# nelpy/ghost

Measured on AMD Instinct MI355X. Metric: Msamples/s CWT (128ch x 1e6 samp x 100 scales); % HBM roofline; 1/2/4/8 GPU, higher is better.
Workload: dtype f32

## Files before the change

ghost_amd/csrc/api.cpp:

```cpp
#include <hip/hip_runtime.h>

#include <algorithm>
#include <cmath>
#include <cstdio>
#include <cstdlib>
#include <cstring>
#include <exception>
#include <map>
#include <new>
#include <string>
#include <vector>

#include "../../include/ghostcwt.h"
#include "../../include/ghostcwt_debug.h"
#include <memory>

#include "errors.h"
#include "host_out.h"
#include "interp.h"
#include "kernels.h"
#include "morse_exact.h"
#include "morlet_exact.h"
#include "options.h"
#include "planner.h"
// ... 12 lines not shown

int hip_err(hipError_t e, const char* what) {
  g_err = std::string(what) + ": " + hipGetErrorString(e);
  return e == hipErrorOutOfMemory ? GCWT_ERR_NOMEM : GCWT_ERR_HIP;
}

#define HIP_TRY(call)                                  \
  do {                                                 \
    hipError_t e_ = (call);                            \
    if (e_ != hipSuccess) return hip_err(e_, #call);   \
  } while (0)

struct EpochDev {
  SynthItemDev* items = nullptr;
  int n_items = 0;
  SynthLevelDev* levels = nullptr;
  Synth7Item* items7 = nullptr;
  Synth7Level* levels7 = nullptr;
  int n_items7 = 0;
  Synth7Item* items7w = nullptr;
  int n_items7w = 0;
  Synth7Item* items7n = nullptr;
  int n_items7n = 0;
  SynthiItem* items_i = nullptr;
  SynthiLevel* levels_i = nullptr;
  int n_items_i = 0;
  SynthpItem* items_p[2] = {nullptr, nullptr};
  SynthpLevel* levels_p = nullptr;
  int n_items_p[2] = {0, 0};
  PredLevel* pred_levels = nullptr;
};

constexpr int64_t kFullbandCacheBytes = (int64_t)16 << 30;

enum Stage { ST_MEAN = 0, ST_FWD, ST_DECIM, ST_BLOCK, ST_SYNTH, ST_DIRECT, ST_FULLBAND, ST_INTERP, ST_BLOCKCONV, ST_COUNT };

}

struct gcwt_plan {
  HostPlan hp;
  bool uploaded = false;
  int profiling = 0;
  int synth_cols = 32;
  int synth7_narrow_r = 2;
  bool fuse_blocks = true;
  int synth_kernel = 7;
  bool prune_inputs = true;
  bool fast_fft = true;
  int drop_stores = 0;
  bool clock_probe = false;
  bool use_synth16 = false;
  int device = -1;
  hipStream_t stream = nullptr;
  hipStream_t aux[2] = {nullptr, nullptr};
  bool level_streams = true;
  bool use_synthp = false;
  bool use_graphs = true;
  bool fullband4 = true;
  int fullband_group = 0;
  int64_t fullband_cache_cap = 0;
  bool hfull_cache_full = false;
  int synth7_order = 0;
  int synthp_help = -1;
  int synthp_lgnb = -1;
  int interp_lgnb = -1;
  int interp_grid = -1;
  bool last_fold = false;
// ... 102 lines not shown

template <typename T>
int upload_vec(T** p, const std::vector<T>& v, hipStream_t st) {
  int rc = dev_alloc(p, v.size());
  if (rc) return rc;
  if (!v.empty()) HIP_TRY(hipMemcpyAsync(*p, v.data(), v.size() * sizeof(T), hipMemcpyHostToDevice, st));
  return GCWT_OK;
}

void free_dev(gcwt_plan* p) {
  auto fr = [](auto*& q) { if (q) { (void)hipFree((void*)q); q = nullptr; } };
  fr(p->d_y); fr(p->d_tw64); fr(p->d_x); fr(p->d_xr); fr(p->d_xb); fr(p->d_xs); fr(p->d_probe); fr(p->d_amps); fr(p->d_z); fr(p->d_hfull); fr(p->d_bank); fr(p->d_gain); fr(p->d_gain_lv); fr(p->d_half_tw); fr(p->d_psi); fr(p->d_psi_tail); fr(p->d_psi_lit); fr(p->d_tw4096);
  fr(p->d_tw256); fr(p->d_level_tw); fr(p->d_sums); fr(p->d_scale_list); fr(p->d_scale_aux); fr(p->d_interp_coef); fr(p->d_bank_sc); fr(p->d_direct_sc); fr(p->d_bc_h); fr(p->d_bc_rows); fr(p->d_bc_x); fr(p->d_bc_tw);
  fr(p->d_in);
  if (p->d_out) { (void)hipFree(p->d_out); p->d_out = nullptr; }
  if (p->h_pred) { (void)hipHostFree(p->h_pred); p->h_pred = nullptr; }
  fr(p->d_hist); fr(p->d_bands); fr(p->d_pred); fr(p->d_scale_level); fr(p->d_scale_length); fr(p->d_run_mask);
  for (gcwt_plan*& sub : p->sub_plan)
    if (sub) { gcwt_plan_destroy(sub); sub = nullptr; }
  for (auto& kv : p->hfull_cache) (void)hipFree(kv.second);
  p->hfull_cache.clear();
  p->hfull_cache_bytes = 0;
  p->host_out.release();
  for (auto& e : p->ep_dev) { fr(e.items); fr(e.levels); fr(e.items7); fr(e.items7w); fr(e.items7n); fr(e.levels7); fr(e.items_i); fr(e.levels_i); fr(e.items_p[0]); fr(e.items_p[1]); fr(e.levels_p); fr(e.pred_levels); }
  p->ep_dev.clear();
  if (p->graph_exec) { (void)hipGraphExecDestroy(p->graph_exec); p->graph_exec = nullptr; }
  for (auto e : p->ev_pool) (void)hipEventDestroy(e);
  p->ev_pool.clear();
  if (p->stream) { (void)hipStreamDestroy(p->stream); p->stream = nullptr; }
  for (auto& q : p->aux) if (q) { (void)hipStreamDestroy(q); q = nullptr; }
  if (p->det_stream) { (void)hipStreamDestroy(p->det_stream); p->det_stream = nullptr; }
  p->uploaded = false;
}

int get_event(gcwt_plan* p, hipEvent_t* e) {
  if (p->ev_used == p->ev_pool.size()) {
    hipEvent_t n;
    HIP_TRY(hipEventCreate(&n));
    p->ev_pool.push_back(n);
  }
  *e = p->ev_pool[p->ev_used++];
  return GCWT_OK;
}

enum LevelKernel { LK_SYNTH16 = 0, LK_SYNTH7 = 7, LK_INTERP = 9 };
inline bool level_pipelined(const gcwt_plan* p, const LevelPlan& lp) {
  return p->use_synthp && lp.interp_q == 2 && lp.interp_factor >= 4 && lp.interp_factor <= kSynthpMaxFactor &&
// ... 110 lines not shown
      return set_err(GCWT_ERR_INVALID, "a destination that is not page-locked takes dense rows (dst_pitch = row_elems)");
    HIP_TRY(rows_to_host(d_src, src_pitch, n_rows, row_elems, dst, dst_pitch, (flags & GCWT_OUT_F64) != 0,
                         (flags & GCWT_HOST_PINNED) != 0));
    return (int)GCWT_OK;
  });
}

static int gcwt_plan_create_impl(gcwt_plan** out, const gcwt_params* params) {
  if (!out || !params) return set_err(GCWT_ERR_INVALID, "NULL argument");
  *out = nullptr;
  std::unique_ptr<gcwt_plan> owner(new (std::nothrow) gcwt_plan());
  gcwt_plan* p = owner.get();
  if (!p) return set_err(GCWT_ERR_NOMEM, "out of host memory");
  std::string err;
  int rc = build_host_plan(*params, &p->hp, &err);
  if (rc != GCWT_OK) return set_err(rc, err);
  p->hp.prm.freqs_hz = p->hp.freqs.data();
  p->hp.prm.epoch_bounds = p->hp.bounds.data();
  p->hp.prm.n_epochs = (int32_t)(p->hp.bounds.size() / 2);
  p->device = params->device;
  p->high_precision = p->hp.high_precision;
  p->use_synth16 = option_or("synth16", 0) == 1;
  p->synth_cols = option_or("synth_cols", 32) == 16 ? 16 : 32;
  p->synth7_narrow_r = (int)option_or("synth7_narrow_r", 2);
  p->fuse_blocks = option_or("fuse_blocks", 1) != 0;
  p->prune_inputs = option_or("prune_inputs", 1) != 0;
  p->fast_fft = option_or("slow_fft", 0) == 0;
  p->level_streams = option_or("level_streams", 1) != 0;
  if (option_is_set("interp_grid")) p->interp_grid = option_or("interp_grid", 0) != 0;
  p->synth_streams = option_or("synth_streams", 0) != 0;
  p->fold_mean = option_or("fold_mean", 1) != 0;
  p->interp_lgnb = (int)option_or("interp_lgnb", -1);
  p->use_synthp = kMeasureBuild && option_or("synthp", 0) != 0;
  p->synthp_lgnb = (int)option_or("synthp_lgnb", -1);
  p->synthp_help = (int)option_or("synthp_help", -1);
  p->use_graphs = option_or("graphs", 1) != 0;
  p->synth7_order = (int)option_or("synth7_order", 0);
  p->auto_threshold = 1e-9f * (float)option_or("auto_threshold_ppb", 1500);
  p->kappa_eps = 1e-9f * (float)option_or("auto_kappa_ppb", 160);
  p->oob_tol = 1e-12f * (float)option_or("auto_oob_ppt", 25000);
  p->fullband_group = (int)option_or("fullband_group", 0);
  p->fullband4 = option_or("fullband4", 1) != 0;
  p->synth_kernel = kMeasureBuild && option_or("synth_kernel", 7) == 8 ? 8 : 7;
  p->drop_stores = kMeasureBuild && option_is_set("synth_drop_stores") ? (int)std::max<long long>(1, option_or("synth_drop_stores", 1)) : 0;
  p->clock_probe = kMeasureBuild && option_is_set("clock_probe");
  for (const auto& s : p->hp.scales)
    if (s.method == GCWT_SCALE_DIRECT) p->max_direct_len = std::max(p->max_direct_len, s.length);
// ... 273 lines not shown
  if ((rc = upload_vec(&p->d_interp_coef, hp.interp_coef, p->stream))) return bail(rc);
  p->n_listed = (int)scale_list.size();
  {
    const size_t n = ((size_t)p->n_listed + 8) * 256 * (hp.morlet ? 2 : 1);
    if ((rc = dev_alloc(&p->d_gain_lv, n))) return bail(rc);
    hipError_t hz = hipMemsetAsync(p->d_gain_lv, 0, sizeof(float) * n, p->stream);
    if (hz != hipSuccess) return bail(hip_err(hz, "gain rows reset"));
  }
  p->ep_dev.resize(hp.epochs.size());
  for (size_t e = 0; e < hp.epochs.size(); ++e) {
    const EpochPlan& ep = hp.epochs[e];
    if (ep.batch_count == 0) continue;
    std::vector<SynthItemDev> items;
    for (size_t i = 0; i < ep.items.size(); ++i)
      if (level_kernel(p, hp.levels[ep.items[i].level]) == LK_SYNTH16)
        items.push_back({ep.items[i].level, ep.items[i].scale, ep.items[i].blk0, ep.items[i].nblk});
    p->ep_dev[e].n_items = (int)items.size();
    std::vector<SynthLevelDev> lv(hp.levels.size());
    for (size_t l = 0; l < lv.size(); ++l)
      lv[l] = {hp.levels[l].decimation, hp.levels[l].hop, hp.levels[l].halo, ep.lv[l].blk_lo,
               ep.lv[l].xb_offset, hp.levels[l].twiddle_offset};
    if ((rc = upload_vec(&p->ep_dev[e].items, items, p->stream))) return bail(rc);
    if ((rc = upload_vec(&p->ep_dev[e].levels, lv, p->stream))) return bail(rc);
    std::vector<Synth7Item> items7, items7w, items7n;
    std::vector<Synth7Level> lv7(hp.levels.size());
    for (size_t l = 0; l < lv7.size(); ++l) {
      const LevelPlan& lp = hp.levels[l];
      int lg = 0;
      while ((1 << lg) < lp.decimation) ++lg;
      lv7[l] = {lp.decimation, lg, lp.hop, lp.halo, ep.lv[l].nblk, (int32_t)lp.scales.size(),
                scale_off[l], ep.lv[l].blk_lo, n_plain[l], (int32_t)(l * 256), lp.band_shift, 0, ep.lv[l].xb_offset,
                lp.twiddle_offset, ep.lv[l].xr_offset, ep.lv[l].m - 1};
      const bool narrow = lp.halo <= 48 && lp.decimation <= p->synth7_narrow_r && p->synth_cols == 32;
      const int cols = narrow ? 16 : p->synth_cols;
      const int bpb = std::max(1, cols / lp.decimation);
      const int n_rtiles = std::max(1, lp.decimation / cols);
      if (level_kernel(p, lp) != LK_SYNTH7) continue;
      for (int b0 = 0; b0 < ep.lv[l].nblk; b0 += bpb)
        for (int rt = 0; rt < n_rtiles; ++rt) (lp.halo > 48 ? items7w : narrow ? items7n : items7).push_back({(int32_t)l, b0, rt, 0});
    }
    if (p->synth7_order == 1) std::reverse(items7.begin(), items7.end());
    else if (p->synth7_order == 2) {
      std::vector<std::vector<Synth7Item>> by(hp.levels.size());
      for (const auto& it : items7) by[(size_t)it.level].push_back(it);
      std::vector<Synth7Item> mixed;
      std::vector<double> pos(by.size(), 0.0);
      size_t left = items7.size();
      while (left) {
        size_t best = by.size(); double frac = 2.0;
        for (size_t l = 0; l < by.size(); ++l)
          if (pos[l] < (double)by[l].size() && pos[l] / (double)by[l].size() < frac) { frac = pos[l] / (double)by[l].size(); best = l; }
        mixed.push_back(by[best][(size_t)pos[best]]);
        pos[best] += 1.0; --left;
      }
      items7.swap(mixed);
    }
    p->ep_dev[e].n_items7 = (int)items7.size();
    p->ep_dev[e].n_items7w = (int)items7w.size();
    p->ep_dev[e].n_items7n = (int)items7n.size();
    if ((rc = upload_vec(&p->ep_dev[e].items7n, items7n, p->stream))) return bail(rc);
    if ((rc = upload_vec(&p->ep_dev[e].items7, items7, p->stream))) return bail(rc);
    if ((rc = upload_vec(&p->ep_dev[e].items7w, items7w, p->stream))) return bail(rc);
    if ((rc = upload_vec(&p->ep_dev[e].levels7, lv7, p->stream))) return bail(rc);
    std::vector<SynthiItem> items_i;
    std::vector<std::pair<int, int>> pending;
    std::vector<SynthiLevel> lvi(hp.levels.size());
    std::vector<int> order;
    std::vector<int> order_p;
    for (size_t l = 0; l < hp.levels.size(); ++l)
      if (level_kernel(p, hp.levels[l]) == LK_INTERP)
        (level_pipelined(p, hp.levels[l]) ? order_p : order).push_back((int)l);
    std::sort(order.begin(), order.end(),
              [&](int x, int y) { return hp.levels[x].decimation > hp.levels[y].decimation; });
    std::sort(order_p.begin(), order_p.end(),
              [&](int x, int y) { return hp.levels[x].decimation > hp.levels[y].decimation; });
    for (int l : order) {
      const LevelPlan& lp = hp.levels[l];
      int lgq = 0;
      while ((1 << lgq) < lp.interp_q) ++lgq;
      int lgnb = lp.decimation <= 32 && lp.interp_q <= 2 ? 1 : 0;
      if (p->interp_lgnb >= 0) lgnb = std::min(p->interp_lgnb, 2);
      while (lgnb > 0 && (lp.interp_q << lgnb) > kInterpMaxPhases) --lgnb;
// ... 369 lines not shown
        RUN(ST_DECIM, launch_level_small(p->d_x, xr, n1, q, kRowLen, P, hp.max_xr, p->d_tw4096, slots, ls, taper));
      }
      const float scale = (float)(1.0 / ((double)hp.block * (double)Pt));
      const LevelKernel lk = level_kernel(p, lp);
      if (lk == LK_SYNTH16 || (lk == LK_SYNTH7 && !fused_blocks))
        RUN(ST_BLOCK, launch_block_fft(xr, p->d_xb + el.xb_offset, el.m, lp.hop, lp.halo, el.blk_lo,
                                       el.nblk, hp.max_xr, hp.max_xb, p->d_tw256, scale, slots, ls));
    }
    if (side) {
      p->cur = nullptr;
      for (int k = 0; k < 2; ++k) {
        if (!forked[k]) continue;
        hipEvent_t done;
        int rc_ = get_event(p, &done);
        if (rc_) return rc_;
        he = hipEventRecord(done, p->aux[k]);
        if (he == hipSuccess) he = hipStreamWaitEvent(st, done, 0);
        if (he != hipSuccess) return hip_err(he, "level streams join");
      }
    }
    const EpochDev& dev = p->ep_dev[ep.batch_first];
    hipStream_t si = st;
    if (dev.n_items_i > 0) {
      const bool beside = p->synth_streams && (dev.n_items7 > 0 || dev.n_items7w > 0 || dev.n_items7n > 0 || dev.n_items > 0);
      if (beside) {
        hipEvent_t levels_done;
        int rc_ = get_event(p, &levels_done);
        if (rc_) return rc_;
        he = hipEventRecord(levels_done, st);
        if (he == hipSuccess) he = hipStreamWaitEvent(p->aux[0], levels_done, 0);
        if (he != hipSuccess) return hip_err(he, "synthesis fork");
        si = p->aux[0];
      }
      SynthiArgs ai{};
      ai.tw256 = p->d_tw256;
      ai.level_tw = p->d_level_tw;
      ai.items = dev.items_i;
      ai.levels = dev.levels_i;
      ai.scale_list = p->d_scale_list;
      ai.scale_aux = p->d_scale_aux;
      ai.gain = p->d_gain;
      ai.coef = p->d_interp_coef;
      ai.out = dout;
      ai.row_len = row_len;
      ai.xr = p->d_xr;
      ai.xr_cstride = hp.max_xr;
      ai.xb_scale = (float)(1.0 / ((double)hp.block * (double)Pt));
// ... 32 lines not shown
#ifdef GCWT_MEASURE
      if (strided) return set_err(GCWT_ERR_UNSUPPORTED, "output stride with the pipelined interpolating kernel");
      RUN(ST_INTERP, launch_synthp(mode, ap, dev.n_items_p[k], slots, k == 1, si));
#else
      return set_err(GCWT_ERR_INVALID, "internal: a level planned for the measure build's pipelined kernel");
#endif
      p->cur = nullptr;
    }
    if (dev.n_items > 0) {
      SynthArgs a{};
      a.xb = p->d_xb;
      a.bank = p->d_bank;
      a.tw256 = p->d_tw256;
      a.level_tw = p->d_level_tw;
      a.items = dev.items;
      a.levels = dev.levels;
      a.out = dout;
      a.xb_cstride = hp.max_xb;
      a.row_len = row_len;
      a.n_scales = S;
      a.seg = sout;
      RUN(ST_SYNTH, launch_synth(mode, a, dev.n_items, slots, st));
    }
    for (int variant = 0; variant < 3; ++variant) {
      const int wide = variant == 2;
      const int cols7 = variant == 0 ? 16 : p->synth_cols;
      const int n7 = variant == 0 ? dev.n_items7n : wide ? dev.n_items7w : dev.n_items7;
      if (n7 == 0) continue;
      Synth7Args a7{};
      a7.xb = p->d_xb;
      a7.bank = p->d_bank;
      a7.tw256 = p->d_tw256;
      a7.level_tw = p->d_level_tw;
      a7.items = variant == 0 ? dev.items7n : wide ? dev.items7w : dev.items7;
      a7.levels = dev.levels7;
      a7.scale_list = p->d_scale_list;
      a7.gain = p->d_gain;
      a7.gain_lv = p->d_gain_lv;
      a7.level_half_tw = p->d_half_tw;
      a7.complex_gains = hp.morlet ? 1 : 0;
      a7.out = dout;
      a7.xb_cstride = hp.max_xb;
      a7.row_len = row_len;
      a7.n_scales = S;
      a7.drop_stores = p->drop_stores;
      a7.seg = sout;
      a7.clock_probe = p->d_probe;
      if (fused_blocks) {
        a7.xr = p->d_xr;
        a7.xr_cstride = hp.max_xr;
        a7.xb_scale = (float)(1.0 / ((double)hp.block * (double)Pt));
      }
      if (strided) {
        RUN(ST_SYNTH, launch_synth7s(mode, cols7, a7, n7, slots, st));
        continue;
      }
#ifdef GCWT_MEASURE
      if (p->synth_kernel == 8 && variant == 1)
        RUN(ST_SYNTH, launch_synth8(mode, p->synth_cols, a7, n7, slots, st));
      else
#endif
        RUN(ST_SYNTH, launch_synth7(mode, cols7, wide != 0, a7, n7, slots, st));
    }
    if (si != st) {
      hipEvent_t interp_done;
      int rc_ = get_event(p, &interp_done);
      if (rc_) return rc_;
      he = hipEventRecord(interp_done, si);
      if (he == hipSuccess) he = hipStreamWaitEvent(st, interp_done, 0);
      if (he != hipSuccess) return hip_err(he, "synthesis join");
    }
    if (p->detect && p->d_y) {
      hipEvent_t pred_done;
      int rc_ = get_event(p, &pred_done);
      if (rc_) return rc_;
      he = hipEventRecord(pred_done, p->det_stream);
      if (he == hipSuccess) he = hipStreamWaitEvent(st, pred_done, 0);
// ... 698 lines not shown
```

ghost_amd/csrc/kernels.h:

```cpp
#pragma once
#include <hip/hip_runtime.h>

#include <algorithm>
#include <cstdint>

#include "../../include/ghostcwt.h"

namespace gcwt {

constexpr int kRowLenDev = 4096;

#ifdef GCWT_MEASURE
constexpr bool kMeasureBuild = true;
#else
constexpr bool kMeasureBuild = false;
#endif

struct BankScale {
  double omega;
  double half_delay;
  int64_t length;
  int64_t amp_offset;
  int32_t bin_lo, n_bins;
  int32_t decimation;
// ... 101 lines not shown
  const float2* tw256;
  const float2* level_tw;
  const Synth7Item* items;
  const Synth7Level* levels;
  const int32_t* scale_list;
  const float* gain;
  const float* gain_lv;
  const float2* level_half_tw;
  float* out;
  int64_t xb_cstride;
  int64_t row_len;
  const float2* xr;
  int64_t xr_cstride;
  float xb_scale;
  int32_t complex_gains;
  unsigned long long* clock_probe;
  int32_t n_scales;
  int32_t drop_stores;
  SegOut seg;
};

hipError_t launch_synth7(int mode, int ncol, bool wide_halo, const Synth7Args& a, int n_items, int n_channels,
                         hipStream_t st);
hipError_t launch_synth7s(int mode, int ncol, const Synth7Args& a, int n_items, int n_channels, hipStream_t st);

struct SynthiItem {
  int32_t level, blk0;
  int32_t pass0, n_pass;
  int32_t wt_lo, wt_hi;
};
struct SynthiLevel {
  int32_t decimation, q, log2q, factor;
  int32_t hop, halo, nblk, n_scales, scale_offset, blk_base;
  int32_t log2nb, taps;
  int64_t tw_offset;
  int64_t xr_offset;
  int64_t m_mask;
  int64_t coef_offset;
};
struct SynthiArgs {
  const float2* tw256;
  const float2* level_tw;
  const SynthiItem* items;
  const SynthiLevel* levels;
  const int32_t* scale_list;
  const int32_t* scale_aux;
// ... 204 lines not shown
```

ghost_amd/csrc/options.cpp:

```cpp
#include "options.h"

#include <cctype>
#include <cstdlib>
#include <cstring>
#include <map>
#include <mutex>
#include <string>

#include "kernels.h"

namespace gcwt {
namespace {

const char* const kSelect[] = {"synth16", "synth_cols", "fuse_blocks", "slow_fft", "level_streams", "interp_grid",
                               "synth_streams", "interp_lgnb", "merge_levels", "split_levels", "interp",
                               "batch_bytes", "stage_floats", "fullband_group", "blockconv",
                               "direct_max_len", "graphs", "plan_threads", "fullband_cache_mb", "auto_threshold_ppb", "auto_kappa_ppb", "auto_oob_ppt", "synth7_order", "host_widen", "host_threads", "fullband4", "cu_count", "synth7_narrow_r", "fold_mean"};
const char* const kMeasureOnly[] = {"halo_margin", "interp_q", "interp_taps", "interp_min_r", "prune_inputs", "clock_phases",
                                    "synth_kernel", "synth_drop_stores", "clock_probe", "synthi_pad_kb",
                                    "synthp", "synthp_lgnb", "synthp_help"};
const char* const kEnvBudgets[] = {"batch_bytes", "stage_floats"};

std::mutex g_mu;
std::map<std::string, long long>& table() {
  static std::map<std::string, long long> t;
  return t;
}

template <size_t N>
bool in_list(const char* name, const char* const (&list)[N]) {
  for (const char* s : list)
    if (!strcmp(s, name)) return true;
  return false;
}

bool from_env(const char* name, long long* v) {
  std::string var = "GHOSTCWT_";
  for (const char* c = name; *c; ++c) var.push_back((char)toupper((unsigned char)*c));
  const char* e = getenv(var.c_str());
  if (!e) return false;
  *v = *e ? atoll(e) : 1;
// ... 38 lines not shown
```

ghost_amd/csrc/planner.cpp:

```cpp
#include "planner.h"
#include "interp.h"
#include "morse_exact.h"
#include "morlet_exact.h"
#include "options.h"

#include <algorithm>
#include <climits>
#include <cstdlib>
#include <cmath>
#include <map>
#include <atomic>
#include <mutex>
#include <new>
#include <thread>

namespace gcwt {

static int exact_method(const HostPlan& hp, int64_t length) {
  if (length <= hp.direct_max_len) return GCWT_SCALE_DIRECT;
  if (length <= hp.blockconv_max_len) return GCWT_SCALE_BLOCKCONV;
  return GCWT_SCALE_FULLBAND;
}
static bool uses_segment_fft(int method) { return method == GCWT_SCALE_SPECTRAL || method == GCWT_SCALE_FULLBAND; }

// ... 29 lines not shown
  if (rebalance) {
    double taps = 0.0, best = rest[0] / hp->bc_fill;
    for (int k = 1; k <= n && hp->scales[order[k - 1]].length <= kDirectMaxLen; ++k) {
      taps += (double)hp->scales[order[k - 1]].length;
      const double c = taps / kTapsPerUnit + rest[k] / hp->bc_fill;
      if (c < best) { best = c; first = k; }
    }
    for (int k = 0; k < first; ++k) hp->scales[order[k]].method = GCWT_SCALE_DIRECT;
  }
  for (int start = first; start < n; start = stop[start]) {
    HostPlan::BcGroup g;
    g.first = start - first;
    g.count = stop[start] - start;
    geometry(stop[start] - 1, &g.hop, &g.back);
    g.ramp = ramp;
    hp->bc_groups.push_back(g);
  }
  order.erase(order.begin(), order.begin() + first);
  hp->n_blockconv = (int)order.size();
  for (int k = 0; k < hp->n_blockconv; ++k) hp->scales[order[k]].blockconv_index = k;
}

static int halo_margin() { return (int)std::max<long long>(0, option_or("halo_margin", 2)); }

double morse_log_gain(double u, double gamma, double beta) {
  return beta * std::log(u) - (beta / gamma) * (std::pow(u, gamma) - 1.0);
}

static void band_edges(double gamma, double beta, double eps, double* u_lo, double* u_hi) {
  const double target = std::log(eps);
  double lo = 1e-9, hi = 1.0;
  for (int i = 0; i < 200; ++i) {
    double mid = 0.5 * (lo + hi);
    if (morse_log_gain(mid, gamma, beta) < target) lo = mid; else hi = mid;
  }
  *u_lo = lo;
  lo = 1.0; hi = 64.0;
  for (int i = 0; i < 200; ++i) {
    double mid = 0.5 * (lo + hi);
    if (morse_log_gain(mid, gamma, beta) < target) hi = mid; else lo = mid;
  }
  *u_hi = hi;
}

namespace {
struct MorletBand { double xi_hi = 0, xi_neg = 0, xi_lo = 0, t_support = 0; };
// ... 494 lines not shown
    for (const ScalePlan& sp : hp->scales)
      if (uses_segment_fft(sp.method)) l = std::max(l, sp.length);
    return l;
  };
  for (int round = 0; round < 4; ++round) {
    const int64_t lmax = longest_fft_kernel();
    int64_t pmin = INT64_MAX;
    for (int e = 0; e < n_ep; ++e)
      pmin = std::min(pmin, std::min(pmax, fft_of(hp->bounds[2 * e], hp->bounds[2 * e + 1], lmax)));
    const int r_cap = (int)std::min<int64_t>(kMaxDecimation, pmin / B);
    bool moved = false;
    for (ScalePlan& sp : hp->scales) {
      if (sp.method != GCWT_SCALE_SPECTRAL) continue;
      const bool two_sided = sp.theta_neg > 0.0;
      auto fits = [&](int r) {
        if (!two_sided) return sp.theta_hi * (double)r <= 2.0 * M_PI;
        if (r > kMaxTwoPassDecimation) return false;
        const int g = std::max(1, r / 16);
        return (sp.theta_hi + sp.theta_neg) * (double)r + 2.0 * M_PI * (double)(g + 1) / (double)B <= 2.0 * M_PI;
      };
      int r = 2;
      while (2 * r <= r_cap && fits(2 * r)) r *= 2;
      sp.decimation = r;
      int halo = std::max((int)std::ceil(sp.support / (double)r) + halo_margin(), 16);
      if (r == 2) halo += halo & 1;
      if (B - 2 * halo < 32 || (two_sided && !fits(2))) {
        sp.method = exact_method(*hp, sp.length);
        moved = true;
      }
    }
    for (int pass = 0; pass < 64; ++pass) {
      std::map<int, std::vector<int>> by_r;
      for (int i = 0; i < prm.n_freqs; ++i)
        if (hp->scales[i].method == GCWT_SCALE_SPECTRAL) by_r[hp->scales[i].decimation].push_back(i);
      bool changed = false;
      for (auto& kv : by_r) {
        bool any_two_sided = false;
        for (int i : kv.second) any_two_sided = any_two_sided || hp->scales[i].theta_neg > 0.0;
        if (!any_two_sided) continue;
        const int r = kv.first, g = std::max(1, r / 16);
        const double delta = 2.0 * M_PI / ((double)B * r);
        int shift = 0, worst = -1;
        double worst_need = 0.0;
        for (int i : kv.second) shift = std::max(shift, (int)std::ceil(hp->scales[i].theta_neg / delta));
        shift = (shift + g - 1) / g * g;
        for (int i : kv.second) {
          const double need = std::max(hp->scales[i].theta_hi / delta - (double)(B - shift), 0.0);
          if (need > 0.0 && need >= worst_need) { worst_need = need; worst = i; }
        }
        if (worst < 0) continue;
        int widest = worst;
        for (int i : kv.second)
          if (hp->scales[i].theta_neg + hp->scales[i].theta_hi >
              hp->scales[widest].theta_neg + hp->scales[widest].theta_hi) widest = i;
        ScalePlan& sp = hp->scales[widest];
        changed = true;
        if (r == 2) {
          sp.method = exact_method(*hp, sp.length);
          moved = true;
        } else {
          sp.decimation = r / 2;
          int halo = std::max((int)std::ceil(sp.support / (double)(r / 2)) + halo_margin(), 16);
          if (r / 2 == 2) halo += halo & 1;
          if (B - 2 * halo < 32) {
            sp.method = exact_method(*hp, sp.length);
            moved = true;
          }
        }
        break;
      }
      if (!changed) break;
    }
    if (!moved) break;
  }
  {
    std::map<int, std::vector<int>> by_r;
    for (int i = 0; i < prm.n_freqs; ++i)
      if (hp->scales[i].method == GCWT_SCALE_SPECTRAL) by_r[hp->scales[i].decimation].push_back(i);
    for (auto& kv : by_r) {
      bool shifted = false;
      for (int i : kv.second) shifted = shifted || hp->scales[i].theta_neg > 0.0;
      if (!shifted) continue;
      for (size_t n = 256; n < kv.second.size(); ++n) {
        ScalePlan& sp = hp->scales[kv.second[n]];
        sp.method = exact_method(*hp, sp.length);
      }
    }
  }
  {
    if (option_or("merge_levels", 1) != 0) {
      std::map<int, std::vector<int>> by_r;
      for (int i = 0; i < prm.n_freqs; ++i)
        if (hp->scales[i].method == GCWT_SCALE_SPECTRAL) by_r[hp->scales[i].decimation].push_back(i);
      auto halo_of = [&](int r, const std::vector<int>& idx) {
        int h = 16;
        for (int i : idx) {
          int hs = std::max((int)std::ceil(hp->scales[i].support / (double)r) + halo_margin(), 16);
          if (r == 2) hs += hs & 1;
          h = std::max(h, hs);
        }
        return h;
      };
      const double kPrologue = 3.0;
      auto cost = [&](int r, const std::vector<int>& idx) {
        return (kPrologue + (double)idx.size()) / (double)(B - 2 * halo_of(r, idx));
      };
      std::vector<int> rs;
      for (const auto& kv : by_r) rs.push_back(kv.first);
      for (size_t k = rs.size(); k-- > 1;) {
        const int r = rs[k], r_lo = r / 2;
        if (r_lo < 2 || !by_r.count(r_lo) || by_r[r].empty() || by_r[r_lo].empty()) continue;
        std::vector<int> merged = by_r[r_lo];
        merged.insert(merged.end(), by_r[r].begin(), by_r[r].end());
        if (merged.size() > 256 || halo_of(r_lo, merged) > 32) continue;
        if (cost(r_lo, merged) < cost(r, by_r[r]) + cost(r_lo, by_r[r_lo])) {
          for (int i : by_r[r]) hp->scales[i].decimation = r_lo;
          by_r[r_lo] = merged;
          by_r[r].clear();
        }
      }
    }
  }
// ... 42 lines not shown
      return fail(GCWT_ERR_UNSUPPORTED,
                  "longest wavelet is too long for time blocks of 2^max_fft_log2 samples");
    for (int64_t c0 = e0; c0 < e1;) {
      const int64_t c1 = std::min(e1, (c0 + core_len) & ~(int64_t)63);
      const int64_t u0 = c0 - halo_s, u1 = c1 + halo_s;
      const int64_t in0 = u0 - ramp > e0 ? u0 - ramp : e0, in1 = u1 + ramp < e1 ? u1 + ramp : e1;
      add(in0, in1, c0, c1, pmax, in0 > e0 ? u0 : -1, in1 < e1 ? u1 : -1);
      c0 = c1;
    }
  }
  const int n_seg = (int)hp->epochs.size();
  (void)n_seg;

  const int r_cap = (int)std::min<int64_t>(kMaxDecimation, pmin / B);
  bool split = false;
  split = option_or("split_levels", 0) == 1;
  std::map<std::pair<int, int>, int> level_of;
  std::map<int, int> owner_of_r;
  for (int i = 0; i < prm.n_freqs; ++i) {
    ScalePlan& sp = hp->scales[i];
    if (sp.method != GCWT_SCALE_SPECTRAL) continue;
    const int r = sp.decimation;
    if (r > r_cap) return fail(GCWT_ERR_UNSUPPORTED, "internal: decimation beyond the shortest FFT");
    int halo = std::max((int)std::ceil(sp.support / (double)r) + halo_margin(), 16);
    if (r == 2) halo += halo & 1;
    const std::pair<int, int> key(r, sp.theta_neg > 0.0 && halo > 48 ? 2 : (split && halo > 16 ? 1 : 0));
    auto it = level_of.find(key);
    if (it == level_of.end()) {
      LevelPlan lp;
      lp.decimation = r;
      const int idx = (int)hp->levels.size();
      if (!owner_of_r.count(r)) owner_of_r[r] = idx;
      lp.xr_owner = owner_of_r[r];
      level_of[key] = idx;
      hp->levels.push_back(lp);
      it = level_of.find(key);
    }
    sp.level = it->second;
    LevelPlan& lp = hp->levels[sp.level];
    lp.scales.push_back(i);
    lp.halo = std::max(lp.halo, halo);
  }
  {
    std::map<int, int> shift_of_r;
    for (const LevelPlan& lp : hp->levels) {
      const double delta = 2.0 * M_PI / ((double)B * lp.decimation);
      int& shift = shift_of_r[lp.decimation];
      for (int i : lp.scales)
// ... 169 lines not shown
```

ghost_amd/csrc/synth.hip:

```cpp
#include <hip/hip_runtime.h>

#include "kernels.h"
#include "synth_math.h"

#ifndef GCWT_STORE_AUX
#define GCWT_STORE_AUX 2
#endif

namespace gcwt {

__device__ __forceinline__ v2f phase_carrier(int shift, int r, int R) {
  float sn, cs;
  sincospif(-2.0f * (float)(shift * r) / (256.0f * (float)R), &sn, &cs);
  return (v2f){cs, sn};
}

template <int STRIDE>
__device__ __forceinline__ void twiddle_to_planes(v2f* exw, const v2f (&v)[16], const v2f* tw, int stride = STRIDE) {
  const int st = STRIDE ? STRIDE : stride;
#pragma unroll
  for (int jj = 0; jj < 8; ++jj) {
    const v4f w2 = *reinterpret_cast<const v4f*>(tw + 2 * jj);
    exw[(2 * jj) * st] = jj == 0 ? v[0] : cmulv(v[dft16_pos(2 * jj)], (v2f){w2.x, w2.y});
    exw[(2 * jj + 1) * st] = cmulv(v[dft16_pos(2 * jj + 1)], (v2f){w2.z, w2.w});
// ... 252 lines not shown
    for (int m1 = 1; m1 < 15; ++m1) {
      const v2f z = v[dft16_pos(m1)];
      const bool keep = WIDE ? (keep_rows >> m1) & 1u
                             : m1 == 1 ? keep1 : m1 == 2 ? keep2 : m1 == 13 ? keep13 : m1 == 14 ? keep14 : true;
      const unsigned vo = voff0 + (unsigned)m1 * vstep;
      if (MODE == GCWT_OUT_COMPLEX_C64) {
        typedef unsigned v2u __attribute__((ext_vector_type(2)));
        if (keep) __builtin_amdgcn_raw_buffer_store_b64(__builtin_bit_cast(v2u, z), rsrc, vo, 0, GCWT_STORE_AUX);
      } else {
        const float p2 = __builtin_fmaf(z.y, z.y, z.x * z.x);
        const float val = MODE == GCWT_OUT_AMPLITUDE_F32 ? __builtin_amdgcn_sqrtf(p2) : p2;
        if (keep) __builtin_amdgcn_raw_buffer_store_b32(__builtin_bit_cast(unsigned, val), rsrc, vo, 0, GCWT_STORE_AUX);
      }
    }
  }
  if (kMeasureBuild && a.clock_probe && tid == 0) {
    atomicAdd(a.clock_probe, (unsigned long long)(__builtin_amdgcn_s_memtime() - probe_c0));
    atomicAdd(a.clock_probe + 1, (unsigned long long)(__builtin_amdgcn_s_memrealtime() - probe_t0));
    for (int i = 0; i < 4; ++i) atomicAdd(a.clock_probe + 2 + i, (unsigned long long)(probe_ph[i] - probe_t0));
    atomicAdd(a.clock_probe + 6, 1ull);
  }
}

template <int NCOL, bool WIDE, bool CG>
static hipError_t launch_synth7_n(int mode, const Synth7Args& a, int n_items, int n_channels,
                                  hipStream_t st) {
  constexpr int lds = 16 * (16 * NCOL + 1) * 8 + 16 * 18 * 8 + 8 * 320 * 4 + 256 * 4 + 256 * 8;
  static bool attr_done[64] = {};
  int dev_ = 0;
  (void)hipGetDevice(&dev_);
  bool& attr_set = attr_done[dev_ & 63];
  if (!attr_set) {
    hipError_t e = hipFuncSetAttribute((const void*)k_synth7<GCWT_OUT_AMPLITUDE_F32, NCOL, WIDE, CG>,
                                       hipFuncAttributeMaxDynamicSharedMemorySize, lds);
    if (e != hipSuccess) return e;
    e = hipFuncSetAttribute((const void*)k_synth7<GCWT_OUT_POWER_F32, NCOL, WIDE, CG>,
                            hipFuncAttributeMaxDynamicSharedMemorySize, lds);
    if (e != hipSuccess) return e;
    e = hipFuncSetAttribute((const void*)k_synth7<GCWT_OUT_COMPLEX_C64, NCOL, WIDE, CG>,
                            hipFuncAttributeMaxDynamicSharedMemorySize, lds);
    if (e != hipSuccess) return e;
    attr_set = true;
  }
  dim3 grid(n_items, n_channels), block(16 * NCOL);
  if (mode == GCWT_OUT_AMPLITUDE_F32)
    hipLaunchKernelGGL((k_synth7<GCWT_OUT_AMPLITUDE_F32, NCOL, WIDE, CG>), grid, block, lds, st, a);
// ... 35 lines not shown
```

Measured before the change: 9558.

## Add per-block synth7q kernel for decimation-2 levels with paired even/odd stores

Adds a new synthesis kernel, k_synth7q, for decimation-2 levels with small halo. Each workgroup handles 16 blocks and computes both polyphase components (even and odd) from the same loaded input spectrum, then writes them as interleaved 64-bit stores after a lane transpose. The planner now rounds decimation-2 halos up to a multiple of 8 (through a new measurement-only line_halo option), which lines up with the kernel's store layout. The default synth7_narrow_r changes to 1 so this path runs by default for eligible levels, excluding Morlet, complex output and band-shifted levels. The cost is more code, extra LDS for the twiddle tables, and slightly larger halos that add redundant work.

```diff
diff --git a/ghost_amd/csrc/api.cpp b/ghost_amd/csrc/api.cpp
--- a/ghost_amd/csrc/api.cpp
+++ b/ghost_amd/csrc/api.cpp
@@ -58,6 +58,10 @@
   int n_items7w = 0;
   Synth7Item* items7n = nullptr;
   int n_items7n = 0;
+  Synth7Item* items7q = nullptr;
+  int n_items7q = 0;
+  Synth7Item* items7qn = nullptr;
+  int n_items7qn = 0;
   SynthiItem* items_i = nullptr;
   SynthiLevel* levels_i = nullptr;
   int n_items_i = 0;
@@ -78,7 +82,7 @@
   bool uploaded = false;
   int profiling = 0;
   int synth_cols = 32;
-  int synth7_narrow_r = 2;
+  int synth7_narrow_r = 1;
   bool fuse_blocks = true;
   int synth_kernel = 7;
   bool prune_inputs = true;
@@ -227,7 +231,7 @@
   p->hfull_cache.clear();
   p->hfull_cache_bytes = 0;
   p->host_out.release();
-  for (auto& e : p->ep_dev) { fr(e.items); fr(e.levels); fr(e.items7); fr(e.items7w); fr(e.items7n); fr(e.levels7); fr(e.items_i); fr(e.levels_i); fr(e.items_p[0]); fr(e.items_p[1]); fr(e.levels_p); fr(e.pred_levels); }
+  for (auto& e : p->ep_dev) { fr(e.items); fr(e.levels); fr(e.items7); fr(e.items7w); fr(e.items7n); fr(e.items7q); fr(e.items7qn); fr(e.levels7); fr(e.items_i); fr(e.levels_i); fr(e.items_p[0]); fr(e.items_p[1]); fr(e.levels_p); fr(e.pred_levels); }
   p->ep_dev.clear();
   if (p->graph_exec) { (void)hipGraphExecDestroy(p->graph_exec); p->graph_exec = nullptr; }
   for (auto e : p->ev_pool) (void)hipEventDestroy(e);
@@ -384,7 +388,7 @@
   p->high_precision = p->hp.high_precision;
   p->use_synth16 = option_or("synth16", 0) == 1;
   p->synth_cols = option_or("synth_cols", 32) == 16 ? 16 : 32;
-  p->synth7_narrow_r = (int)option_or("synth7_narrow_r", 2);
+  p->synth7_narrow_r = (int)option_or("synth7_narrow_r", 1);
   p->fuse_blocks = option_or("fuse_blocks", 1) != 0;
   p->prune_inputs = option_or("prune_inputs", 1) != 0;
   p->fast_fft = option_or("slow_fft", 0) == 0;
@@ -704,7 +708,8 @@
                ep.lv[l].xb_offset, hp.levels[l].twiddle_offset};
     if ((rc = upload_vec(&p->ep_dev[e].items, items, p->stream))) return bail(rc);
     if ((rc = upload_vec(&p->ep_dev[e].levels, lv, p->stream))) return bail(rc);
-    std::vector<Synth7Item> items7, items7w, items7n;
+    std::vector<Synth7Item> items7, items7w, items7n, items7q, items7qn;
+    const int narrow_r = p->synth7_narrow_r == 1 ? 2 : p->synth7_narrow_r;
     std::vector<Synth7Level> lv7(hp.levels.size());
     for (size_t l = 0; l < lv7.size(); ++l) {
       const LevelPlan& lp = hp.levels[l];
@@ -713,13 +718,18 @@
       lv7[l] = {lp.decimation, lg, lp.hop, lp.halo, ep.lv[l].nblk, (int32_t)lp.scales.size(),
                 scale_off[l], ep.lv[l].blk_lo, n_plain[l], (int32_t)(l * 256), lp.band_shift, 0, ep.lv[l].xb_offset,
                 lp.twiddle_offset, ep.lv[l].xr_offset, ep.lv[l].m - 1};
-      const bool narrow = lp.halo <= 48 && lp.decimation <= p->synth7_narrow_r && p->synth_cols == 32;
+      const bool narrow = lp.halo <= 48 && lp.decimation <= narrow_r && p->synth_cols == 32;
+      const bool per_block = narrow && p->synth7_narrow_r == 1 && lp.decimation == 2 && lp.halo <= 32 &&
+                             lp.band_shift == 0 && !hp.morlet && hp.prm.out_mode != GCWT_OUT_COMPLEX_C64;
       const int cols = narrow ? 16 : p->synth_cols;
       const int bpb = std::max(1, cols / lp.decimation);
       const int n_rtiles = std::max(1, lp.decimation / cols);
       if (level_kernel(p, lp) != LK_SYNTH7) continue;
       for (int b0 = 0; b0 < ep.lv[l].nblk; b0 += bpb)
-        for (int rt = 0; rt < n_rtiles; ++rt) (lp.halo > 48 ? items7w : narrow ? items7n : items7).push_back({(int32_t)l, b0, rt, 0});
+        for (int rt = 0; rt < n_rtiles; ++rt)
+          (lp.halo > 48 ? items7w : per_block ? items7qn : narrow ? items7n : items7).push_back({(int32_t)l, b0, rt, 0});
+      if (per_block)
+        for (int b0 = 0; b0 < ep.lv[l].nblk; b0 += 16) items7q.push_back({(int32_t)l, b0, 0, 0});
     }
     if (p->synth7_order == 1) std::reverse(items7.begin(), items7.end());
     else if (p->synth7_order == 2) {
@@ -740,6 +750,10 @@
     p->ep_dev[e].n_items7 = (int)items7.size();
     p->ep_dev[e].n_items7w = (int)items7w.size();
     p->ep_dev[e].n_items7n = (int)items7n.size();
+    p->ep_dev[e].n_items7q = (int)items7q.size();
+    p->ep_dev[e].n_items7qn = (int)items7qn.size();
+    if ((rc = upload_vec(&p->ep_dev[e].items7q, items7q, p->stream))) return bail(rc);
+    if ((rc = upload_vec(&p->ep_dev[e].items7qn, items7qn, p->stream))) return bail(rc);
     if ((rc = upload_vec(&p->ep_dev[e].items7n, items7n, p->stream))) return bail(rc);
     if ((rc = upload_vec(&p->ep_dev[e].items7, items7, p->stream))) return bail(rc);
     if ((rc = upload_vec(&p->ep_dev[e].items7w, items7w, p->stream))) return bail(rc);
@@ -1155,7 +1169,7 @@
     const EpochDev& dev = p->ep_dev[ep.batch_first];
     hipStream_t si = st;
     if (dev.n_items_i > 0) {
-      const bool beside = p->synth_streams && (dev.n_items7 > 0 || dev.n_items7w > 0 || dev.n_items7n > 0 || dev.n_items > 0);
+      const bool beside = p->synth_streams && (dev.n_items7 > 0 || dev.n_items7w > 0 || dev.n_items7n > 0 || dev.n_items7q > 0 || dev.n_items > 0);
       if (beside) {
         hipEvent_t levels_done;
         int rc_ = get_event(p, &levels_done);
@@ -1234,17 +1248,19 @@
       a.seg = sout;
       RUN(ST_SYNTH, launch_synth(mode, a, dev.n_items, slots, st));
     }
-    for (int variant = 0; variant < 3; ++variant) {
+    for (int variant = -1; variant < 3; ++variant) {
       const int wide = variant == 2;
-      const int cols7 = variant == 0 ? 16 : p->synth_cols;
-      const int n7 = variant == 0 ? dev.n_items7n : wide ? dev.n_items7w : dev.n_items7;
+      const int cols7 = variant <= 0 ? 16 : p->synth_cols;
+      const int n7 = variant < 0 ? (strided ? dev.n_items7qn : dev.n_items7q)
+                                 : variant == 0 ? dev.n_items7n : wide ? dev.n_items7w : dev.n_items7;
       if (n7 == 0) continue;
       Synth7Args a7{};
       a7.xb = p->d_xb;
       a7.bank = p->d_bank;
       a7.tw256 = p->d_tw256;
       a7.level_tw = p->d_level_tw;
-      a7.items = variant == 0 ? dev.items7n : wide ? dev.items7w : dev.items7;
+      a7.items = variant < 0 ? (strided ? dev.items7qn : dev.items7q)
+                             : variant == 0 ? dev.items7n : wide ? dev.items7w : dev.items7;
       a7.levels = dev.levels7;
       a7.scale_list = p->d_scale_list;
       a7.gain = p->d_gain;
@@ -1265,6 +1281,10 @@
       }
       if (strided) {
         RUN(ST_SYNTH, launch_synth7s(mode, cols7, a7, n7, slots, st));
+        continue;
+      }
+      if (variant < 0) {
+        RUN(ST_SYNTH, launch_synth7q(mode, a7, n7, slots, st));
         continue;
       }
 #ifdef GCWT_MEASURE
diff --git a/ghost_amd/csrc/kernels.h b/ghost_amd/csrc/kernels.h
--- a/ghost_amd/csrc/kernels.h
+++ b/ghost_amd/csrc/kernels.h
@@ -147,6 +147,7 @@
 
 hipError_t launch_synth7(int mode, int ncol, bool wide_halo, const Synth7Args& a, int n_items, int n_channels,
                          hipStream_t st);
+hipError_t launch_synth7q(int mode, const Synth7Args& a, int n_items, int n_channels, hipStream_t st);
 hipError_t launch_synth7s(int mode, int ncol, const Synth7Args& a, int n_items, int n_channels, hipStream_t st);
 
 struct SynthiItem {
diff --git a/ghost_amd/csrc/options.cpp b/ghost_amd/csrc/options.cpp
--- a/ghost_amd/csrc/options.cpp
+++ b/ghost_amd/csrc/options.cpp
@@ -16,7 +16,7 @@
                                "synth_streams", "interp_lgnb", "merge_levels", "split_levels", "interp",
                                "batch_bytes", "stage_floats", "fullband_group", "blockconv",
                                "direct_max_len", "graphs", "plan_threads", "fullband_cache_mb", "auto_threshold_ppb", "auto_kappa_ppb", "auto_oob_ppt", "synth7_order", "host_widen", "host_threads", "fullband4", "cu_count", "synth7_narrow_r", "fold_mean"};
-const char* const kMeasureOnly[] = {"halo_margin", "interp_q", "interp_taps", "interp_min_r", "prune_inputs", "clock_phases",
+const char* const kMeasureOnly[] = {"halo_margin", "line_halo", "interp_q", "interp_taps", "interp_min_r", "prune_inputs", "clock_phases",
                                     "synth_kernel", "synth_drop_stores", "clock_probe", "synthi_pad_kb",
                                     "synthp", "synthp_lgnb", "synthp_help"};
 const char* const kEnvBudgets[] = {"batch_bytes", "stage_floats"};
diff --git a/ghost_amd/csrc/planner.cpp b/ghost_amd/csrc/planner.cpp
--- a/ghost_amd/csrc/planner.cpp
+++ b/ghost_amd/csrc/planner.cpp
@@ -75,6 +75,15 @@
 }
 
 static int halo_margin() { return (int)std::max<long long>(0, option_or("halo_margin", 2)); }
+
+static int block_halo(double support, int r) {
+  int halo = std::max((int)std::ceil(support / (double)r) + halo_margin(), 16);
+  const long long lines = option_or("line_halo", 7);
+  if (r == 2) halo = (lines & 1) ? (halo + 7) & ~7 : halo + (halo & 1);
+  if (r == 4 && (lines & 2)) halo = (halo + 3) & ~3;
+  if (r == 8 && (lines & 4)) halo += halo & 1;
+  return halo;
+}
 
 double morse_log_gain(double u, double gamma, double beta) {
   return beta * std::log(u) - (beta / gamma) * (std::pow(u, gamma) - 1.0);
@@ -615,8 +624,7 @@
       int r = 2;
       while (2 * r <= r_cap && fits(2 * r)) r *= 2;
       sp.decimation = r;
-      int halo = std::max((int)std::ceil(sp.support / (double)r) + halo_margin(), 16);
-      if (r == 2) halo += halo & 1;
+      const int halo = block_halo(sp.support, r);
       if (B - 2 * halo < 32 || (two_sided && !fits(2))) {
         sp.method = exact_method(*hp, sp.length);
         moved = true;
@@ -653,8 +661,7 @@
           moved = true;
         } else {
           sp.decimation = r / 2;
-          int halo = std::max((int)std::ceil(sp.support / (double)(r / 2)) + halo_margin(), 16);
-          if (r / 2 == 2) halo += halo & 1;
+          const int halo = block_halo(sp.support, r / 2);
           if (B - 2 * halo < 32) {
             sp.method = exact_method(*hp, sp.length);
             moved = true;
@@ -688,9 +695,7 @@
       auto halo_of = [&](int r, const std::vector<int>& idx) {
         int h = 16;
         for (int i : idx) {
-          int hs = std::max((int)std::ceil(hp->scales[i].support / (double)r) + halo_margin(), 16);
-          if (r == 2) hs += hs & 1;
-          h = std::max(h, hs);
+          h = std::max(h, block_halo(hp->scales[i].support, r));
         }
         return h;
       };
@@ -779,8 +784,7 @@
     if (sp.method != GCWT_SCALE_SPECTRAL) continue;
     const int r = sp.decimation;
     if (r > r_cap) return fail(GCWT_ERR_UNSUPPORTED, "internal: decimation beyond the shortest FFT");
-    int halo = std::max((int)std::ceil(sp.support / (double)r) + halo_margin(), 16);
-    if (r == 2) halo += halo & 1;
+    const int halo = block_halo(sp.support, r);
     const std::pair<int, int> key(r, sp.theta_neg > 0.0 && halo > 48 ? 2 : (split && halo > 16 ? 1 : 0));
     auto it = level_of.find(key);
     if (it == level_of.end()) {
diff --git a/ghost_amd/csrc/synth.hip b/ghost_amd/csrc/synth.hip
--- a/ghost_amd/csrc/synth.hip
+++ b/ghost_amd/csrc/synth.hip
@@ -298,6 +298,308 @@
   }
 }
 
+#ifndef GCWT_SYNTH_MORLET_TU
+constexpr int kSynth7qHeld = 0;
+
+template <int JHI, bool PH1, bool HALF>
+__device__ __forceinline__ void gain_first_layer_q(v2f v[16], const v2f (&p0)[16], const v2f (&p1)[16], const float4* g,
+                                                   const v2f* wc, const v2f* hl) {
+#pragma unroll
+  for (int q = 0; q < 4; ++q) {
+    if (4 * q >= JHI) continue;
+    const float4 gq = g[q];
+    const float gs[4] = {gq.x, gq.y, gq.z, gq.w};
+#pragma unroll
+    for (int i = 0; i < 4; i += 2) {
+      const int j = 4 * q + i;
+      if (j >= JHI) continue;
+      v2f x0 = p0[j], x1 = p0[j + 1];
+      if (j < kSynth7qHeld) {
+        if (PH1) { x0 = p1[j]; x1 = p1[j + 1]; }
+      } else {
+        if (PH1) {
+          const v4f w2 = *reinterpret_cast<const v4f*>(wc + j);
+          x0 = cmulv(x0, (v2f){w2.x, w2.y});
+          x1 = cmulv(x1, (v2f){w2.z, w2.w});
+        }
+        if (HALF) {
+          const v4f h2 = *reinterpret_cast<const v4f*>(hl + j);
+          x0 = cmulv(x0, (v2f){h2.x, h2.y});
+          x1 = cmulv(x1, (v2f){h2.z, h2.w});
+        }
+      }
+      v[j] = x0 * gs[i];
+      if (j + 1 < JHI) v[j + 1] = x1 * gs[i + 1];
+    }
+  }
+  bfly4_in<(8 >= JHI), (12 >= JHI)>(v[0], v[4], v[8], v[12]);
+  bfly4_in<(9 >= JHI), (13 >= JHI)>(v[1], v[5], v[9], v[13]);
+  bfly4_in<(10 >= JHI), (14 >= JHI)>(v[2], v[6], v[10], v[14]);
+  bfly4_in<(11 >= JHI), (15 >= JHI)>(v[3], v[7], v[11], v[15]);
+}
+
+template <int MODE, bool PH1>
+__device__ __forceinline__ void synth7q_phase(float (&amp)[16], const v2f (&p0)[16], const v2f (&p1)[16], const float4* hs,
+                                              int entry, bool half, const v2f* wc, const v2f* hl, v2f* exw,
+                                              const v2f* exr, const v2f* tw) {
+  v2f v[16];
+  const bool made_half = kSynth7qHeld < 16 && half;
+  switch ((unsigned)entry >> 24) {
+#define GCWT_WINDOW(hi) case 16 - (hi): \
+    if (made_half) gain_first_layer_q<hi, PH1, true>(v, p0, p1, hs, wc, hl); \
+    else gain_first_layer_q<hi, PH1, false>(v, p0, p1, hs, wc, hl); \
+    break;
+    GCWT_WINDOW(15) GCWT_WINDOW(14) GCWT_WINDOW(13) GCWT_WINDOW(12) GCWT_WINDOW(11) GCWT_WINDOW(10) GCWT_WINDOW(9)
+#undef GCWT_WINDOW
+    default:
+      if (made_half) gain_first_layer_q<16, PH1, true>(v, p0, p1, hs, wc, hl);
+      else gain_first_layer_q<16, PH1, false>(v, p0, p1, hs, wc, hl);
+      break;
+  }
+  idft16v_tail(v);
+  twiddle_to_planes<1>(exw, v, tw);
+  __syncthreads();
+#pragma unroll
+  for (int k1 = 0; k1 < 16; ++k1) v[k1] = exr[k1 * 257];
+  __syncthreads();
+  idft16v(v);
+#pragma unroll
+  for (int m1 = 1; m1 < 15; ++m1) {
+    const v2f z = v[dft16_pos(m1)];
+    const float p2 = __builtin_fmaf(z.y, z.y, z.x * z.x);
+    amp[m1] = MODE == GCWT_OUT_AMPLITUDE_F32 ? __builtin_amdgcn_sqrtf(p2) : p2;
+  }
+  amp[0] = amp[15] = 0.f;
+}
+
+__device__ __forceinline__ void transpose_rows16(unsigned (&x)[4]) {
+  const auto s01 = __builtin_amdgcn_permlane16_swap(x[0], x[1], false, false);
+  const auto s23 = __builtin_amdgcn_permlane16_swap(x[2], x[3], false, false);
+  const auto t02 = __builtin_amdgcn_permlane32_swap(s01[0], s23[0], false, false);
+  const auto t13 = __builtin_amdgcn_permlane32_swap(s01[1], s23[1], false, false);
+  x[0] = t02[0]; x[2] = t02[1]; x[1] = t13[0]; x[3] = t13[1];
+}
+
+template <int MODE>
+__global__ void __launch_bounds__(256, 3) k_synth7q(const Synth7Args a) {
+  static_assert(MODE != GCWT_OUT_COMPLEX_C64, "amplitude and power only");
+  static_assert(kSynth7qHeld >= 0 && kSynth7qHeld <= 16 && kSynth7qHeld % 2 == 0, "pairs of operands");
+  constexpr int kThreads = 256, kPlane = kThreads + 1, kChunk = 8, kGainRow = 16 * 20, kTwPitch = 18;
+  extern __shared__ __attribute__((aligned(16))) char smem[];
+  v2f* const ex = reinterpret_cast<v2f*>(smem);
+  v2f* const twl = ex + 16 * kPlane;
+  v2f* const wcl = twl + 16 * kTwPitch;
+  v2f* const hfl = wcl + 16 * kTwPitch;
+  float* const stage = reinterpret_cast<float*>(hfl + 16 * kTwPitch);
+  int* const sc_lds = reinterpret_cast<int*>(stage + kChunk * kGainRow);
+
+  const Synth7Item it = a.items[blockIdx.x];
+  const Synth7Level lv = a.levels[it.level];
+  const int c = blockIdx.y;
+  const int seg = c / a.seg.n_channels, ch = c - seg * a.seg.n_channels;
+  const int hop = lv.hop, halo = lv.halo;
+  {
+    const int64_t span = (int64_t)hop * 2;
+    const int64_t first = (int64_t)(lv.blk_base + it.blk0) * span;
+    const int64_t last = first + 16 * span;
+    if (last <= a.seg.w_lo[seg] || first >= a.seg.w_hi[seg]) return;
+  }
+  const int tid = threadIdx.x;
+  long long probe_c0 = 0, probe_t0 = 0, probe_ph[4] = {0, 0, 0, 0};
+  if (kMeasureBuild && a.clock_probe) { probe_c0 = __builtin_amdgcn_s_memtime(); probe_t0 = __builtin_amdgcn_s_memrealtime(); }
+  const int colw = tid >> 4, t = tid & 15;
+  const int* const scales = a.scale_list + lv.scale_offset;
+  const int sc_v = tid < lv.n_scales ? scales[tid] : 0;
+  const float2 tw_v = a.tw256[(t * colw) & 255];
+  constexpr int kRowVec = 64;
+  const float4* const gain_rows = reinterpret_cast<const float4*>(a.gain_lv + (int64_t)lv.scale_offset * (4 * kRowVec));
+  float4 g_v0, g_v1;
+  const int wave_s = __builtin_amdgcn_readfirstlane(tid >> 6);
+  auto tid_now = [&]() {
+    int ln;
+    asm volatile("v_mbcnt_lo_u32_b32 %0, -1, 0\n\tv_mbcnt_hi_u32_b32 %0, -1, %0" : "=v"(ln));
+    return (wave_s << 6) | ln;
+  };
+  auto load_gains = [&](int b0, int f) {
+    g_v0 = gain_rows[b0 * kRowVec + f];
+    if constexpr (kChunk == 8) g_v1 = gain_rows[b0 * kRowVec + kThreads + f];
+  };
+  auto park_one = [&](int f, const float4& g) {
+    *reinterpret_cast<float4*>(stage + (f >> 6) * kGainRow + ((f >> 2) & 15) * 20 + (f & 3) * 4) = g;
+  };
+  auto park_gains = [&](int f) { park_one(f, g_v0); if constexpr (kChunk == 8) park_one(kThreads + f, g_v1); };
+  load_gains(0, tid);
+  const bool has_half = lv.n_plain < lv.n_scales;
+  const float2 half_v = has_half ? a.level_half_tw[lv.half_offset + t + 16 * colw] : make_float2(1.f, 0.f);
+  const float2* const ltw = a.level_tw + lv.tw_offset;
+  const float2 w_t = ltw[t], w_16 = ltw[16];
+  v2f p0[16], p1[16];
+  auto park_tables = [&]() {
+    if (tid < lv.n_scales) sc_lds[tid] = sc_v;
+    twl[t * kTwPitch + colw] = (v2f){tw_v.x, tw_v.y};
+    hfl[t * kTwPitch + colw] = (v2f){half_v.x, half_v.y};
+    v2f wcur = (v2f){w_t.x, w_t.y};
+    const v2f wstep = (v2f){w_16.x, w_16.y};
+    for (int j = 0; j < colw; ++j) wcur = cmulv(wcur, wstep);
+    wcl[t * kTwPitch + colw] = wcur;
+  };
+  if (a.xr) {
+    v2f* const fx = ex;
+    static_assert(16 * 256 <= 16 * kPlane, "the prologue's exchange must fit the planes");
+    v2f v[16];
+    const int blkx = min(it.blk0 + colw, lv.nblk - 1);
+    const int64_t m_b = (int64_t)(lv.blk_base + blkx) * hop - halo;
+    const float2* xr = a.xr + (int64_t)c * a.xr_cstride + lv.xr_offset;
+#pragma unroll
+    for (int j = 0; j < 16; ++j) {
+      const float2 q = xr[(m_b + t + 16 * j) & lv.m_mask];
+      v[j] = (v2f){q.x, -q.y};
+    }
+    park_tables();
+    park_gains(tid);
+    if (lv.n_scales > kChunk) load_gains(kChunk, tid);
+    if (kMeasureBuild && a.clock_probe) { __builtin_amdgcn_s_waitcnt(0); probe_ph[0] = __builtin_amdgcn_s_memrealtime(); }
+    idft16v(v);
+#pragma unroll
+    for (int m = 0; m < 16; ++m) fx[colw * 256 + t * 16 + (m ^ t)] = v[dft16_pos(m)];
+    __syncthreads();
+    if (kMeasureBuild && a.clock_probe) probe_ph[1] = __builtin_amdgcn_s_memrealtime();
+#pragma unroll
+    for (int k1 = 0; k1 < 16; ++k1) v[k1] = fx[colw * 256 + k1 * 16 + (t ^ k1)];
+#pragma unroll
+    for (int k1 = 1; k1 < 16; ++k1) v[k1] = cmulv(v[k1], twl[t * kTwPitch + k1]);
+    idft16v(v);
+    const float xs = a.xb_scale;
+#pragma unroll
+    for (int j = 0; j < 16; ++j) {
+      const v2f z = v[dft16_pos(j)];
+      p0[j] = (v2f){z.x * xs, -z.y * xs};
+    }
+    if (kMeasureBuild && a.clock_probe) probe_ph[2] = __builtin_amdgcn_s_memrealtime();
+  } else {
+    const int blk = min(it.blk0 + colw, lv.nblk - 1);
+    const float2* xb = a.xb + (int64_t)c * a.xb_cstride + lv.xb_offset + (int64_t)blk * 256 + t;
+#pragma unroll
+    for (int j = 0; j < 16; ++j) {
+      const float2 q = xb[16 * j];
+      p0[j] = (v2f){q.x, q.y};
+    }
+    park_tables();
+    park_gains(tid);
+    if (lv.n_scales > kChunk) load_gains(kChunk, tid);
+  }
+  v2f* const exw = ex + t * kPlane + colw * 16;
+  const v2f* const exr = ex + tid;
+
+  const int64_t n_b = (int64_t)(lv.blk_base + it.blk0) * hop * 2;
+  const int64_t w_lo = a.seg.w_lo[seg];
+  const int64_t w_len = a.seg.w_hi[seg] - w_lo;
+  const unsigned ext_bytes = w_len > 0 && !(kMeasureBuild && (a.drop_stores & 1)) ? (unsigned)(w_len * 4) : 0u;
+  float* const out0 = a.out + ((int64_t)ch * a.n_scales * a.row_len + a.seg.seg_col[seg] + w_lo);
+  const int lane = tid & 63, wv = tid >> 6;
+  const unsigned voff_b0 = (unsigned)(((int)(n_b - w_lo) + (4 * wv * hop + lane - halo) * 2) * 4);
+  const unsigned blk_step = (unsigned)(hop * 2 * 4);
+  const bool keep_lo = lane >= halo, keep_hi = lane < 64 - halo;
+  const bool pair_ok = ext_bytes >= 8;
+  const unsigned pair_lim = pair_ok ? ext_bytes - 8 : 0u;
+  const float4* const st_rd = reinterpret_cast<const float4*>(stage + t * 20);
+  const v2f* const wc_rd = wcl + t * kTwPitch;
+  const v2f* const hf_rd = hfl + t * kTwPitch;
+  __syncthreads();
+#pragma unroll
+  for (int j = 0; j < kSynth7qHeld; ++j) p1[j] = cmulv(p0[j], wc_rd[j]);
+  bool half = false;
+  if (kMeasureBuild && a.clock_probe) probe_ph[3] = __builtin_amdgcn_s_memrealtime();
+
+  for (int b = 0; b < lv.n_scales; ++b) {
+    if (b > 0 && (b & (kChunk - 1)) == 0) {
+      __syncthreads();
+      const int f = tid_now();
+      park_gains(f);
+      if (b + kChunk < lv.n_scales) load_gains(b + kChunk, f);
+      __syncthreads();
+    }
+    if (b == lv.n_plain) {
+      half = true;
+#pragma unroll
+      for (int j = 0; j < kSynth7qHeld; ++j) {
+        const v2f h = hf_rd[j];
+        p0[j] = cmulv(p0[j], h);
+        p1[j] = cmulv(p1[j], h);
+      }
+    }
+    const float4* const hs = st_rd + (b & (kChunk - 1)) * (kGainRow / 4);
+    const int entry = __builtin_amdgcn_readfirstlane(sc_lds[b]);
+    float ev[16], od[16];
+    synth7q_phase<MODE, false>(ev, p0, p1, hs, entry, half, wc_rd, hf_rd, exw, exr, twl + t * kTwPitch);
+    synth7q_phase<MODE, true>(od, p0, p1, hs, entry, half, wc_rd, hf_rd, exw, exr, twl + t * kTwPitch);
+
+    const int srow = entry & kScaleIndexMask;
+    const uint64_t dst_bits = reinterpret_cast<uint64_t>(out0 + (int64_t)srow * a.row_len);
+    const uint32_t dst_lo = __builtin_amdgcn_readfirstlane((uint32_t)dst_bits);
+    const uint32_t dst_hi = __builtin_amdgcn_readfirstlane((uint32_t)(dst_bits >> 32));
+    float* const dst = reinterpret_cast<float*>(((uint64_t)dst_hi << 32) | dst_lo);
+    const __amdgpu_buffer_rsrc_t rsrc = __builtin_amdgcn_make_buffer_rsrc(
+        dst, 0, __builtin_amdgcn_readfirstlane(ext_bytes), 0x00020000);
+#pragma unroll
+    for (int q = 0; q < 4; ++q) {
+      unsigned e[4], o[4];
+#pragma unroll
+      for (int i = 0; i < 4; ++i) {
+        e[i] = __builtin_bit_cast(unsigned, ev[4 * q + i]);
+        o[i] = __builtin_bit_cast(unsigned, od[4 * q + i]);
+      }
+      transpose_rows16(e);
+      transpose_rows16(o);
+      const bool keep = q == 0 ? keep_lo : q == 3 ? keep_hi : true;
+#pragma unroll
+      for (int i = 0; i < 4; ++i) {
+        typedef unsigned v2u __attribute__((ext_vector_type(2)));
+        const unsigned vo = voff_b0 + (unsigned)i * blk_step + (unsigned)(q * 512);
+        if (keep) {
+          if (pair_ok && vo <= pair_lim) {
+            __builtin_amdgcn_raw_buffer_store_b64((v2u){e[i], o[i]}, rsrc, vo, 0, GCWT_STORE_AUX);
+          } else {
+            __builtin_amdgcn_raw_buffer_store_b32(e[i], rsrc, vo, 0, GCWT_STORE_AUX);
+            __builtin_amdgcn_raw_buffer_store_b32(o[i], rsrc, vo + 4u, 0, GCWT_STORE_AUX);
+          }
+        }
+      }
+    }
+  }
+  if (kMeasureBuild && a.clock_probe && tid == 0) {
+    atomicAdd(a.clock_probe, (unsigned long long)(__builtin_amdgcn_s_memtime() - probe_c0));
+    atomicAdd(a.clock_probe + 1, (unsigned long long)(__builtin_amdgcn_s_memrealtime() - probe_t0));
+    for (int i = 0; i < 4; ++i) atomicAdd(a.clock_probe + 2 + i, (unsigned long long)(probe_ph[i] - probe_t0));
+    atomicAdd(a.clock_probe + 6, 1ull);
+  }
+}
+
+hipError_t launch_synth7q(int mode, const Synth7Args& a, int n_items, int n_channels, hipStream_t st) {
+  if (n_items == 0) return hipSuccess;
+  if (mode == GCWT_OUT_COMPLEX_C64 || a.complex_gains) return hipErrorInvalidValue;
+  constexpr int lds = 16 * (16 * 16 + 1) * 8 + 3 * 16 * 18 * 8 + 8 * 320 * 4 + 256 * 4;
+  static bool attr_done[64] = {};
+  int dev_ = 0;
+  (void)hipGetDevice(&dev_);
+  bool& attr_set = attr_done[dev_ & 63];
+  if (!attr_set) {
+    hipError_t e = hipFuncSetAttribute((const void*)k_synth7q<GCWT_OUT_AMPLITUDE_F32>,
+                                       hipFuncAttributeMaxDynamicSharedMemorySize, lds);
+    if (e != hipSuccess) return e;
+    e = hipFuncSetAttribute((const void*)k_synth7q<GCWT_OUT_POWER_F32>, hipFuncAttributeMaxDynamicSharedMemorySize, lds);
+    if (e != hipSuccess) return e;
+    attr_set = true;
+  }
+  dim3 grid(n_items, n_channels), block(256);
+  if (mode == GCWT_OUT_AMPLITUDE_F32)
+    hipLaunchKernelGGL((k_synth7q<GCWT_OUT_AMPLITUDE_F32>), grid, block, lds, st, a);
+  else
+    hipLaunchKernelGGL((k_synth7q<GCWT_OUT_POWER_F32>), grid, block, lds, st, a);
+  return hipGetLastError();
+}
+#endif
+
 template <int NCOL, bool WIDE, bool CG>
 static hipError_t launch_synth7_n(int mode, const Synth7Args& a, int n_items, int n_channels,
                                   hipStream_t st) {
```

Result: no change. 9557 (-0.0%).
